# jwp3/async-multigrid

Measured on AMD Instinct MI355X. Metric: V-cycle iters/sec + fine-grid SpMV HBM GB/s, 512³ 7-pt Laplacian, 1/2/4/8 GPU, higher is better.
Workload: dtype f64

## Files before the change

### async-multigrid_amd/csrc/amg_api.cpp

```cpp
#include <algorithm>
#include <cmath>
#include <cstdlib>
#include <cstdint>
#include <cstring>
#include <mutex>
#include <vector>

#include "amg_async.h"

#include <csignal>
#include <execinfo.h>
#include <unistd.h>

namespace {
struct sigaction g_prev_segv, g_prev_bus, g_prev_abrt;
void amg_fault_trace(int sig, siginfo_t *si, void *uc)
{
   char msg[96];
   const int m = snprintf(msg, sizeof(msg), "[amg] signal %d at address %p, native backtrace:\n", sig, si->si_addr);
   if (m > 0) (void)!write(2, msg, (size_t)m);
   void *buf[64];
   const int n = backtrace(buf, 64);
   backtrace_symbols_fd(buf, n, 2);
   const struct sigaction &prev = sig == SIGSEGV ? g_prev_segv : sig == SIGBUS ? g_prev_bus : g_prev_abrt;
   if ((prev.sa_flags & SA_SIGINFO) && prev.sa_sigaction) {
      prev.sa_sigaction(sig, si, uc);
   } else if (prev.sa_handler != SIG_DFL && prev.sa_handler != SIG_IGN && prev.sa_handler) {
      prev.sa_handler(sig);
   }
   signal(sig, SIG_DFL);
   raise(sig);
}
__attribute__((constructor)) void amg_fault_trace_init()
{
   const char *e = std::getenv("AMG_SEGV_TRACE");
   if (!e || std::atoi(e) == 0) return;
   void *warm[4];
   (void)backtrace(warm, 4);
   struct sigaction sa;
   std::memset(&sa, 0, sizeof(sa));
   sa.sa_sigaction = amg_fault_trace;
   sa.sa_flags = SA_SIGINFO | SA_ONSTACK;
   sigaction(SIGSEGV, &sa, &g_prev_segv);
   sigaction(SIGBUS, &sa, &g_prev_bus);
   sigaction(SIGABRT, &sa, &g_prev_abrt);
}
}

static thread_local std::string g_last_error;

int amg_set_error(int code, const char *fmt, ...)
{
   char buf[1024];
   va_list ap;
   va_start(ap, fmt);
   vsnprintf(buf, sizeof(buf), fmt, ap);
   va_end(ap);
   g_last_error = buf;
   return code;
}

extern "C" const char *amg_last_error(void) { return g_last_error.c_str(); }
extern "C" int amg_version(void) { return 1; }

extern "C" void amg_opts_default(amg_opts *o)
{
   std::memset(o, 0, sizeof(*o));
   o->solver = AMG_MULT;
   o->smoother = AMG_JACOBI;
   o->num_pre_smooth_sweeps = 1;
   o->num_post_smooth_sweeps = 1;
   o->num_fine_smooth_sweeps = 1;
   o->num_coarse_smooth_sweeps = 1;
   o->smooth_weight = 1.0;
   o->num_cycles = 20;
   o->tol = 1e-9;
   o->check_resnorm = 1;
   o->cheby_flag = 0;
   o->num_threads = 1;
   o->jgs_block_rows = 64;
   o->reuse_outer_residual = 0;
   o->async_type = AMG_FULL_ASYNC;
   o->profile = 0;
   o->accel_type = AMG_NO_ACCEL;
   o->cheby_grid = 0;
   o->delay_type = AMG_DELAY_NONE;
   o->delay_usec = 0;
   o->delay_frac = 0.0;
   o->fail_iter = 0;
   o->delay_rank = -1;
   o->max_inflight = 1;
   o->async_comm_save_divisor = 1;
   o->sps_probability_type = AMG_SPS_EXPONENTIAL;
   o->sps_alpha = 1.0;
   o->sps_min_prob = 0.0;
   o->delay_level = -1;
}

extern "C" int amg_init(amg_ctx **out, int device, int nstreams)
{
   AMG_ARG(out, "amg_init: null out");
   int ndev = 0;
   AMG_HIP(hipGetDeviceCount(&ndev));
   AMG_ARG(device >= 0 && device < ndev, "amg_init: device %d of %d", device, ndev);
   AMG_HIP(hipSetDevice(device));
   amg_ctx *c = new amg_ctx();
   c->device = device;
   AMG_HIP(hipStreamCreateWithFlags(&c->stream, hipStreamNonBlocking));
   {
      int least = 0, greatest = 0;
      const char *v = std::getenv("AMG_COMM_PRIORITY");
      const bool hi = v && std::atoi(v) != 0;
      if (hi && hipDeviceGetStreamPriorityRange(&least, &greatest) == hipSuccess && greatest != least) {
         AMG_HIP(hipStreamCreateWithPriority(&c->comm_stream, hipStreamNonBlocking, greatest));
      } else {
         (void)hipGetLastError();
         AMG_HIP(hipStreamCreateWithFlags(&c->comm_stream, hipStreamNonBlocking));
      }
   }
   for (int i = 0; i < std::max(0, nstreams); i++) {
      hipStream_t s;
      AMG_HIP(hipStreamCreateWithFlags(&s, hipStreamNonBlocking));
      c->level_streams.push_back(s);
   }
   AMG_HIP(hipMalloc(&c->d_scalars, 8192 * sizeof(double)));
   AMG_HIP(hipMemset(c->d_scalars, 0, 8192 * sizeof(double)));
   AMG_HIP(hipMalloc(&c->d_err, 64));
   AMG_HIP(hipMemset(c->d_err, 0, 64));
   AMG_HIP(hipHostMalloc(&c->h_pinned, 1024 * sizeof(double)));
   hipDeviceProp_t prop;
   if (hipGetDeviceProperties(&prop, device) == hipSuccess) c->num_cus = prop.multiProcessorCount;
   if (hipDeviceGetAttribute(&c->wall_khz, hipDeviceAttributeWallClockRate, device) != hipSuccess || c->wall_khz <= 0)
      c->wall_khz = 100000;
   if (const char *v = std::getenv("AMG_VALUE_INDEX")) c->value_index = std::atoi(v) != 0;
   if (const char *v = std::getenv("AMG_DICT_INDEX")) c->dict_index = std::atoi(v) != 0;
   if (const char *v = std::getenv("AMG_ROW_PATTERN")) c->row_pattern = std::atoi(v) != 0;
   if (const char *v = std::getenv("AMG_PAIR_PATTERN")) c->pair_pattern = std::min(2, std::max(0, std::atoi(v)));
   if (const char *v = std::getenv("AMG_MASTER_PATTERN")) c->master_pattern = std::atoi(v) != 0;
   if (const char *v = std::getenv("AMG_PAIR_ANCHOR16")) c->pair_anchor16 = std::atoi(v) != 0;
   if (const char *v = std::getenv("AMG_PLANE_MARCH")) {
      c->plane_march = std::atoi(v) > 0;
      if (std::atoi(v) > 1) c->mz_zc = std::min(std::atoi(v), 64), c->mz_zc_auto = 0;
   }
   if (const char *v = std::getenv("AMG_PLANE_MARCH_XCD")) c->mz_xcd = std::atoi(v) != 0;
   if (const char *v = std::getenv("AMG_FUSE_TRANSFER")) c->fuse_transfer = std::atoi(v) != 0;
   if (const char *v = std::getenv("AMG_FUSE_XFER")) c->fuse_xfer = std::atoi(v) != 0;
   if (const char *v = std::getenv("AMG_GRAPHS")) c->graphs = std::atoi(v) != 0;
   if (const char *v = std::getenv("AMG_LONG_FORM")) c->long_form = std::max(0, std::min(2, std::atoi(v)));
   if (const char *v = std::getenv("AMG_LONG_XCD")) c->long_xcd = std::atoi(v) != 0;
   if (const char *v = std::getenv("AMG_OUTER_SLAB")) c->outer_slab = std::max(1, std::atoi(v));
   if (const char *v = std::getenv("AMG_FUSE_OUTER")) c->fuse_outer = std::max(0, std::min(3, std::atoi(v)));
   if (const char *v = std::getenv("AMG_FUSE_XFP_SLAB")) c->fuse_xfp_slab = std::atoi(v) != 0;
   if (const char *v = std::getenv("AMG_FUSE_PROLONG")) c->fuse_prolong = std::max(0, std::min(7, std::atoi(v)));
   if (const char *v = std::getenv("AMG_JGS_SMALL")) c->jgs_small = std::max(0, std::min(2, std::atoi(v)));
   if (const char *v = std::getenv("AMG_JGS_WAVE")) c->jgs_wave = std::max(0, std::min(3, std::atoi(v)));
   if (const char *v = std::getenv("AMG_JGS_FOLD")) c->jgs_fold = std::atoi(v) != 0;
   if (const char *v = std::getenv("AMG_BSR3")) c->bsr3 = std::max(0, std::min(std::atoi(v), 2));
   if (const char *v = std::getenv("AMG_BSR3_XS")) c->bsr3_xs = std::atoi(v) != 0;
   if (const char *v = std::getenv("AMG_MZ_EDGE")) c->mz_edge = std::atoi(v) != 0;
   if (const char *v = std::getenv("AMG_MZ27_OCC")) c->mz27_occ = std::max(-1, std::min(8, std::atoi(v)));
   if (const char *v = std::getenv("AMG_MZ_OCC")) c->mz_occ = std::max(-1, std::min(8, std::atoi(v)));
   if (const char *v = std::getenv("AMG_MZ_PF")) c->mz_pf = std::atoi(v) == 2 ? 2 : (std::atoi(v) == 1 ? 1 : 3);
   if (const char *v = std::getenv("AMG_MZ27_PF")) c->mz27_pf = std::atoi(v) == 1 ? 1 : (std::atoi(v) == 3 ? 3 : 2);
   if (const char *v = std::getenv("AMG_RR_LINES")) c->rr_lines = std::atoi(v) == 2 ? 2 : 1;
   if (const char *v = std::getenv("AMG_RR_OCC")) c->rr_occ = std::atoi(v);
   if (const char *v = std::getenv("AMG_RR_FPF")) c->rr_fpf = std::atoi(v);
   if (const char *v = std::getenv("AMG_RR_ZC")) c->rr_zc = std::max(0, std::min(std::atoi(v), 32));
   if (const char *v = std::getenv("AMG_RR_RING")) c->rr_ring = std::atoi(v) != 0;
   if (const char *v = std::getenv("AMG_MZ_NT")) c->mz_nt = std::atoi(v) & 3;
   if (const char *v = std::getenv("AMG_MZ_LINES")) c->mz_lines = std::atoi(v) == 4 ? 4 : std::atoi(v) == 2 ? 2 : 1;
   if (const char *v = std::getenv("AMG_MZ_LINES_GEMV"))
      c->mz_lines_gemv = std::atoi(v) == 4 ? 4 : std::atoi(v) == 2 ? 2 : 1;
   *out = c;
   return AMG_OK;
}

std::recursive_mutex &amg_teardown_mutex()
{
   static std::recursive_mutex m;
   return m;
}

extern "C" int amg_finalize(amg_ctx *c)
{
   if (!c) return AMG_OK;
   std::lock_guard<std::recursive_mutex> td(amg_teardown_mutex());
   hipSetDevice(c->device);
   hipStreamSynchronize(c->stream);
   if (c->comm_stream) hipStreamSynchronize(c->comm_stream);
   for (auto s : c->level_streams) {
      hipStreamSynchronize(s);
      hipStreamDestroy(s);
   }
   if (c->comm_stream) hipStreamDestroy(c->comm_stream);
   hipStreamDestroy(c->stream);
   hipFree(c->d_partials);
   hipFree(c->d_scalars);
   hipFree(c->d_err);
   hipHostFree(c->h_pinned);
   delete c;
   return AMG_OK;
}

extern "C" int amg_device_errors(amg_ctx *c, int *flags)
{
   AMG_ARG(c && flags, "amg_device_errors: null argument");
   int h[16];
   AMG_HIP(hipStreamSynchronize(c->stream));
   AMG_HIP(hipMemcpy(h, c->d_err, sizeof(h), hipMemcpyDeviceToHost));
   AMG_HIP(hipMemset(c->d_err, 0, sizeof(h)));
   *flags = h[0];
   return AMG_OK;
}

extern "C" int amg_sync(amg_ctx *c)
{
   AMG_ARG(c, "amg_sync: null ctx");
   AMG_HIP(hipStreamSynchronize(c->stream));
   return AMG_OK;
}

int amg_ctx_partials(amg_ctx *c, size_t n, double **out)
{
   if (n > c->partials_cap) {
      AMG_HIP(hipStreamSynchronize(c->stream));
      hipFree(c->d_partials);
      c->d_partials = nullptr;
      size_t cap = std::max<size_t>(n, 1 << 16);
      AMG_HIP(hipMalloc(&c->d_partials, cap * sizeof(double)));
      c->partials_cap = cap;
   }
   *out = c->d_partials;
   return AMG_OK;
}

static int mat_alloc(amg_ctx *c, int nrows, int ncols, long long nnz, amg_mat **out)
{
   amg_mat *A = new amg_mat();
   A->ctx = c;
   A->nrows = nrows;
   A->ncols = ncols;
   A->nnz = nnz;
   size_t np = (size_t)nnz + AMG_NNZ_PAD;
   hipError_t e = hipMalloc(&A->rowptr, ((size_t)nrows + 1) * sizeof(int));
   if (e == hipSuccess) e = hipMalloc(&A->col, np * sizeof(int));
   if (e == hipSuccess) e = hipMalloc(&A->val, np * sizeof(double));
   if (e == hipSuccess) e = hipMalloc(&A->diag, std::max(1, nrows) * sizeof(double));
   if (e != hipSuccess) {
      hipFree(A->rowptr); hipFree(A->col); hipFree(A->val); hipFree(A->diag);
      delete A;
      return amg_set_error(AMG_ERR_OOM, "amg_csr_register: device allocation of %lld nnz failed: %s",
                           nnz, hipGetErrorString(e));
   }
   AMG_HIP(hipMemsetAsync(A->col + nnz, 0, AMG_NNZ_PAD * sizeof(int), c->stream));
   AMG_HIP(hipMemsetAsync(A->val + nnz, 0, AMG_NNZ_PAD * sizeof(double), c->stream));
   *out = A;
   return AMG_OK;
}

static int build_value_index(amg_mat *A)
{
   amg_ctx *c = A->ctx;
   hipStream_t s = c->stream;
   constexpr int NS = 4096;
   unsigned long long *slots = nullptr;
   AMG_HIP(hipMalloc(&slots, NS * sizeof(unsigned long long) + 64));
   int *count = reinterpret_cast<int *>(slots + NS);
   AMG_HIP(hipMemsetAsync(slots, 0xff, NS * sizeof(unsigned long long), s));
   AMG_HIP(hipMemsetAsync(count, 0, sizeof(int), s));
   amgk::vi_collect(s, A->val, A->nnz, slots, NS, count);
   std::vector<unsigned long long> h(NS);
   int cnt = 0;
   AMG_HIP(hipMemcpyAsync(h.data(), slots, NS * sizeof(unsigned long long), hipMemcpyDeviceToHost, s));
   AMG_HIP(hipMemcpyAsync(&cnt, count, sizeof(int), hipMemcpyDeviceToHost, s));
   AMG_HIP(hipStreamSynchronize(s));
   if (cnt < 1 || cnt > 256) {
      hipFree(slots);
      return AMG_OK;
   }
   std::vector<unsigned long long> keys;
   for (auto k : h)
      if (k != ~0ULL) keys.push_back(k);
   std::sort(keys.begin(), keys.end());
   const int T = (int)keys.size();
   std::vector<double> tab(256, 0.0);
   std::memcpy(tab.data(), keys.data(), T * sizeof(double));
   hipError_t e = hipMalloc(&A->vidx, (size_t)A->nnz + 64);
   if (e == hipSuccess) e = hipMalloc(&A->vtab, 256 * sizeof(double));
   if (e != hipSuccess) {
      hipFree(A->vidx);
      hipFree(A->vtab);
      A->vidx = nullptr;
      A->vtab = nullptr;
      hipFree(slots);
      (void)hipGetLastError();
      return AMG_OK;
   }
   AMG_HIP(hipMemcpyAsync(slots, keys.data(), T * sizeof(unsigned long long), hipMemcpyHostToDevice, s));
   AMG_HIP(hipMemcpyAsync(A->vtab, tab.data(), 256 * sizeof(double), hipMemcpyHostToDevice, s));
   AMG_HIP(hipMemsetAsync(A->vidx + A->nnz, 0, 64, s));
   amgk::vi_encode(s, A->val, A->nnz, slots, T, A->vidx);
   AMG_HIP(hipStreamSynchronize(s));
   hipFree(slots);
   A->vi_n = T;
// ... 433 lines not shown
   A->mz_xlo = A->mz_xhi = -1;
}

int amg_mat_finish(amg_mat *A)
{
   amgk::extract_diag(A->ctx->stream, A);
   AMG_HIP(hipGetLastError());
   {
      int *d = nullptr;
      AMG_HIP(hipMalloc(&d, 2 * sizeof(int)));
      AMG_HIP(hipMemsetAsync(d, 0, 2 * sizeof(int), A->ctx->stream));
      amgk::row_max(A->ctx->stream, A, d);
      amgk::diag_uniform(A->ctx->stream, A, d + 1);
      int h[2] = {0, 0};
      double d0 = 0.0;
      hipError_t e = hipMemcpyAsync(h, d, 2 * sizeof(int), hipMemcpyDeviceToHost, A->ctx->stream);
      if (e == hipSuccess && A->nrows > 0)
         e = hipMemcpyAsync(&d0, A->diag, sizeof(double), hipMemcpyDeviceToHost, A->ctx->stream);
      if (e == hipSuccess) e = hipStreamSynchronize(A->ctx->stream);
      hipFree(d);
      if (e != hipSuccess) return amg_set_error(AMG_ERR_HIP, "amg_mat_finish: %s", hipGetErrorString(e));
      A->maxrow = h[0];
      A->diag_uni = A->nrows > 0 && h[1] == 0;
      A->diag_u = d0;
   }
   if (A->ctx->value_index && A->nnz > 0) AMG_TRY(build_value_index(A));
   if (A->ctx->dict_index && A->vidx) AMG_TRY(build_dict_index(A));
   if (A->ctx->row_pattern && A->didx) AMG_TRY(build_row_pattern(A));
   const bool pp = A->dc_maxrow <= 8 || A->nrows >= AMG_PP_LONG_MIN_ROWS || A->ctx->pair_pattern == 2;
   const bool try27 = !pp && A->ctx->plane_march && A->ctx->master_pattern;
   if (A->ctx->pair_pattern && A->rpat && A->dc_maxrow <= AMG_PP_MAXROW && (pp || try27))
      AMG_TRY(build_pair_pattern(A));
   if (A->ctx->master_pattern && A->ppat) AMG_TRY(build_master_pattern(A));
   if (try27 && A->ppat && !A->mz27 && !A->pbase) drop_pair_forms(A);
   return AMG_OK;
}

extern "C" int amg_set_row_pattern(amg_ctx *c, int enable)
{
   AMG_ARG(c, "amg_set_row_pattern: null context");
   c->knob_gen++;
   c->row_pattern = enable ? 1 : 0;
   return AMG_OK;
}

extern "C" int amg_mat_row_pattern(const amg_mat *A)
{
   return A ? A->rp_n : 0;
}

extern "C" int amg_set_pair_pattern(amg_ctx *c, int enable)
{
   AMG_ARG(c, "amg_set_pair_pattern: null context");
   c->knob_gen++;
   c->pair_pattern = enable < 0 ? 0 : enable > 2 ? 2 : enable;
   return AMG_OK;
}

extern "C" int amg_mat_pair_pattern(const amg_mat *A)
{
   return A ? A->pp_n : 0;
}

extern "C" int amg_set_pair_anchor16(amg_ctx *c, int enable)
{
   AMG_ARG(c, "amg_set_pair_anchor16: null context");
   c->knob_gen++;
   c->pair_anchor16 = enable ? 1 : 0;
   return AMG_OK;
}

extern "C" int amg_mat_pair_anchor16(const amg_mat *A)
{
   return (A && A->pdelta) ? 1 : 0;
}

extern "C" int amg_set_master_pattern(amg_ctx *c, int enable)
{
   AMG_ARG(c, "amg_set_master_pattern: null context");
   c->knob_gen++;
   c->master_pattern = enable ? 1 : 0;
   return AMG_OK;
}

extern "C" int amg_mat_master_pattern(const amg_mat *A)
{
   return A ? A->mp_J * (A->mp_uni ? -1 : 1) : 0;
}

extern "C" int amg_set_plane_march(amg_ctx *c, int enable, int zc, int xcd)
{
   AMG_ARG(c, "amg_set_plane_march: null context");
   AMG_ARG(zc >= -1 && zc <= 64, "amg_set_plane_march: planes per chunk %d outside [1, 64] (0: keep, -1: auto)",
           zc);
   c->knob_gen++;
   c->plane_march = enable ? 1 : 0;
   if (zc > 0) c->mz_zc = zc, c->mz_zc_auto = 0;
   if (zc == -1) c->mz_zc = 16, c->mz_zc_auto = 1;
   if (xcd >= 0) c->mz_xcd = xcd ? 1 : 0;
   return AMG_OK;
}

extern "C" int amg_set_jgs_wave(amg_ctx *c, int enable)
{
   AMG_ARG(c, "amg_set_jgs_wave: null context");
   c->knob_gen++;
   c->jgs_wave = std::max(0, std::min(3, enable));
   return AMG_OK;
}

extern "C" int amg_set_jgs_small(amg_ctx *c, int form)
{
   AMG_ARG(c, "amg_set_jgs_small: null context");
   c->knob_gen++;
   c->jgs_small = std::max(0, std::min(2, form));
   return AMG_OK;
}

extern "C" int amg_set_jgs_fold(amg_ctx *c, int enable)
{
   AMG_ARG(c, "amg_set_jgs_fold: null context");
   c->knob_gen++;
   c->jgs_fold = enable != 0;
   return AMG_OK;
}

extern "C" int amg_set_fuse_prolong(amg_ctx *c, int enable)
{
   AMG_ARG(c, "amg_set_fuse_prolong: null context");
   c->knob_gen++;
   c->fuse_prolong = std::max(0, std::min(7, enable));
   return AMG_OK;
}

extern "C" int amg_set_march_lines(amg_ctx *c, int lines)
{
   AMG_ARG(c && (lines == 1 || lines == 2 || lines == 4), "amg_set_march_lines: lines must be 1, 2 or 4");
   c->knob_gen++;
   c->mz_lines = lines;
   c->mz_lines_gemv = lines;
   return AMG_OK;
}

extern "C" int amg_set_march_lines_gemv(amg_ctx *c, int lines)
{
   AMG_ARG(c && (lines == 1 || lines == 2 || lines == 4), "amg_set_march_lines_gemv: lines must be 1, 2 or 4");
   c->knob_gen++;
   c->mz_lines_gemv = lines;
   return AMG_OK;
}

extern "C" int amg_set_fuse_outer(amg_ctx *c, int mode)
{
   AMG_ARG(c && mode >= 0 && mode <= 3, "amg_set_fuse_outer: mode 0, 1, 2 or 3");
   c->knob_gen++;
   c->fuse_outer = mode;
   return AMG_OK;
}

extern "C" int amg_set_outer_slab(amg_ctx *c, int planes)
{
   AMG_ARG(c && planes >= 1, "amg_set_outer_slab: planes must be >= 1");
   c->knob_gen++;
   c->outer_slab = planes;
   return AMG_OK;
}

extern "C" int amg_set_long_form(amg_ctx *c, int form, int xcd)
{
   AMG_ARG(c && form >= 0 && form <= 2, "amg_set_long_form: form 0, 1 or 2");
   c->knob_gen++;
   c->long_form = form;
   c->long_xcd = xcd != 0;
   return AMG_OK;
}

extern "C" int amg_set_graphs(amg_ctx *c, int enable)
{
   AMG_ARG(c, "amg_set_graphs: null context");
   c->knob_gen++;
   c->graphs = enable != 0;
   return AMG_OK;
}

extern "C" int amg_set_march_tuning(amg_ctx *c, int mz_pf, int mz27_pf, int mz_occ, int mz27_occ)
{
   AMG_ARG(c, "amg_set_march_tuning: null context");
   AMG_ARG(mz_pf == -2 || (mz_pf >= 1 && mz_pf <= 3), "amg_set_march_tuning: 7-pt prefetch distance %d", mz_pf);
   AMG_ARG(mz27_pf == -2 || mz27_pf == 1 || mz27_pf == 2 || mz27_pf == 3,
           "amg_set_march_tuning: 27-pt prefetch distance %d (3: the LDS plane ring)",
           mz27_pf);
   AMG_ARG(mz_occ >= -2 && mz_occ <= 8 && mz27_occ >= -2 && mz27_occ <= 8,
           "amg_set_march_tuning: occupancy %d / %d outside [-1, 8]", mz_occ, mz27_occ);
   c->knob_gen++;
   if (mz_pf != -2) c->mz_pf = mz_pf;
   if (mz27_pf != -2) c->mz27_pf = mz27_pf;
   if (mz_occ != -2) c->mz_occ = mz_occ;
   if (mz27_occ != -2) c->mz27_occ = mz27_occ;
   return AMG_OK;
}

extern "C" int amg_set_fuse_transfer(amg_ctx *c, int enable)
{
   AMG_ARG(c, "amg_set_fuse_transfer: null context");
   c->knob_gen++;
   c->fuse_transfer = enable ? 1 : 0;
   return AMG_OK;
}

extern "C" int amg_mat_plane_march(const amg_mat *A)
{
   return A ? A->mz_P : 0;
}

extern "C" int amg_mat_march_points(const amg_mat *A)
{
   return (A && A->mz_P) ? (A->mz27 ? 27 : 7) : 0;
}

extern "C" int amg_set_dict_index(amg_ctx *c, int enable)
{
   AMG_ARG(c, "amg_set_dict_index: null context");
   c->knob_gen++;
   c->dict_index = enable ? 1 : 0;
   return AMG_OK;
}

extern "C" int amg_mat_dict_index(const amg_mat *A)
{
   return A ? A->dc_n : 0;
}

extern "C" int amg_set_value_index(amg_ctx *c, int enable)
{
   AMG_ARG(c, "amg_set_value_index: null context");
   c->knob_gen++;
   c->value_index = enable ? 1 : 0;
   return AMG_OK;
}

extern "C" int amg_mat_value_index(const amg_mat *A)
{
   return A ? A->vi_n : 0;
}

int amg_mat_create_device(amg_ctx *c, int nrows, int ncols, long long nnz, amg_mat **out)
{
   return mat_alloc(c, nrows, ncols, nnz, out);
}

static int build_bsr3(amg_mat *A, const int *rowptr, const int *col, const double *val)
{
   const int n = A->nrows, nb = n / 3;
   if (!A->ctx->bsr3 || n % 3 || n != A->ncols || !A->diag_first || n < 3 || A->nnz < 24LL * n) return AMG_OK;
   std::vector<int> bptr(nb + 1, 0), bdiag(nb, -1), bcol;
   std::vector<unsigned char> mode(nb, 1);
   std::vector<long long> src;
   std::vector<int> js;
   long long blocked = 0;
   for (int t = 0; t < nb; t++) {
      bptr[t + 1] = bptr[t];
      const int r0 = 3 * t;
      const int len = rowptr[r0 + 1] - rowptr[r0];
      if (len < 3 || len % 3) continue;
      bool ok = true;
      js.clear();
      for (int c = 0; c < 3 && ok; c++) {
         const int r = r0 + c, b = rowptr[r], e = rowptr[r + 1];
         ok = e - b == len && col[b] == r;
         int prev = -1, k = b + 1;
         std::vector<int> cols;
         cols.reserve(len);
         bool ins = false;
         for (int q = 0; q < len - 1 && ok; q++, k++) {
            const int cc = col[k];
            if (!ins && r < cc) cols.push_back(r), ins = true;
            ok = cc > prev && cc != r;
            prev = cc;
            cols.push_back(cc);
         }
         if (!ins) cols.push_back(r);
         for (int q = 0; q < len && ok; q += 3) {
            ok = cols[q] % 3 == 0 && cols[q + 1] == cols[q] + 1 && cols[q + 2] == cols[q] + 2;
            if (ok && c == 0) js.push_back(cols[q] / 3);
            if (ok && c > 0) ok = js[q / 3] == cols[q] / 3;
         }
      }
      if (!ok) continue;
      mode[t] = 0;
      blocked++;
      for (size_t q = 0; q < js.size(); q++) {
         if (js[q] == t) bdiag[t] = bptr[t + 1];
         bcol.push_back(js[q]);
         bptr[t + 1]++;
      }
      if (bdiag[t] < 0) return AMG_OK;
      const size_t base = src.size();
      src.resize(base + js.size() * 9, -1);
      for (int c = 0; c < 3; c++) {
         const int r = r0 + c, b = rowptr[r], e = rowptr[r + 1];
         for (int k = b; k < e; k++) {
            const int j = col[k] / 3, cc = col[k] % 3;
            const size_t q = std::lower_bound(js.begin(), js.end(), j) - js.begin();
            src[base + q * 9 + 3 * c + cc] = k;
         }
      }
   }
// ... 619 lines not shown
```

### async-multigrid_amd/csrc/amg_internal.h

```cpp
#pragma once

#include <hip/hip_runtime.h>

#include <cstdarg>
#include <cstdint>
#include <cstdio>
#include <functional>
#include <string>
#include <limits>
#include <vector>

#include "amg_mi355x.h"

int amg_set_error(int code, const char *fmt, ...);

#define AMG_HIP(call)                                                                      \
   do {                                                                                    \
      hipError_t _e = (call);                                                              \
      if (_e != hipSuccess)                                                                \
         return amg_set_error(AMG_ERR_HIP, "%s:%d %s -> %s", __FILE__, __LINE__, #call,   \
                              hipGetErrorString(_e));                                      \
   } while (0)

#define AMG_TRY(call)                                                                      \
   do {                                                                                    \
      int _s = (call);                                                                     \
      if (_s != AMG_OK) return _s;                                                         \
   } while (0)

#define AMG_ARG(cond, ...)                                                                 \
   do {                                                                                    \
      if (!(cond)) return amg_set_error(AMG_ERR_ARG, __VA_ARGS__);                         \
   } while (0)

constexpr int AMG_TILE_ROWS = 256;
constexpr int AMG_CHUNK = 2048;
constexpr int AMG_NNZ_PAD = 8;
constexpr int AMG_DC_MAXROW = 32;
constexpr int AMG_RP_STRIDE = 36;
constexpr int AMG_PP_MAXROW = 32;
constexpr int AMG_PP_LDS = 32 * 1024;
constexpr int AMG_PP_LONG_MIN_ROWS = 1 << 22;
inline int amg_pp_stride(int maxrow) { return 1 + 2 * (maxrow <= 8 ? 8 : AMG_PP_MAXROW); }

constexpr int AMG_PP_NDA = 16;
constexpr int AMG_PP_DA0 = 8;
constexpr int AMG_PP_NK = 256 * 257 * AMG_PP_NDA;
constexpr double AMG_PP_MAXFILL = 1.15;
constexpr int AMG_RPP_OPT = 2;
constexpr int AMG_MP_MAXJ = 32;
constexpr int AMG_MP_LDS = 48 * 1024;

struct amg_transport;

struct amg_ctx {
   amg_transport *xport = nullptr;
   long long replicate_rows = 1LL << 18;
   int device = 0;
   hipStream_t stream = nullptr;
   std::vector<hipStream_t> level_streams;
   hipStream_t comm_stream = nullptr;
   double *d_partials = nullptr;
   size_t partials_cap = 0;
   double *d_scalars = nullptr;
   int *d_err = nullptr;
   double *h_pinned = nullptr;
   int num_cus = 256;
   int wall_khz = 100000;
   int value_index = 1;
   int dict_index = 1;
   int row_pattern = 1;
   int pair_pattern = 1;
   int master_pattern = 1;
   int pair_anchor16 = 0;
   int plane_march = 1;
   int mz_zc = 16;
   int mz_edge = 1;
   int mz_zc_auto = 1;
   int mz27_occ = -1;
   int mz_occ = 0;
   int mz_pf = 3;
   int mz27_pf = 2;
   int mz_xcd = 1;
   int fuse_transfer = 1;
   int bsr3 = 2;
   unsigned knob_gen = 0;
   int graphs = 0;
   int fuse_xfer = 1;
   int fuse_xfp_slab = 0;
   int fuse_prolong = 0;
   int bsr3_xs = 1;
   int fuse_outer = 0;
   int outer_slab = 32;
   int rr_lines = 1;
   int mz_lines = 1;
   int mz_lines_gemv = 2;
   int mz_nt = 0;
   int rr_ring = 0;
   int rr_occ = 0;
   int rr_fpf = 0;
   int long_form = 0;
   int long_xcd = 1;
   int rr_zc = 0;
   int jgs_wave = 1;
   int jgs_small = 2;
   int jgs_fold = 0;
};

struct amg_mat {
   amg_ctx *ctx = nullptr;
   int nrows = 0, ncols = 0;
   long long nnz = 0;
   int *rowptr = nullptr;
   int *col = nullptr;
   double *val = nullptr;
   double *diag = nullptr;
   int diag_first = 1;
   int maxrow = -1;
   amg_mat *trans = nullptr;
   unsigned char *vidx = nullptr;
   double *vtab = nullptr;
   int vi_n = 0;
   unsigned char *didx = nullptr;
   int *doff = nullptr;
   double *dval = nullptr;
   int *danch = nullptr;
   int dc_n = 0;
   int dc_maxrow = 0;
   unsigned char *rpat = nullptr;
   unsigned char *ptab = nullptr;
   int rp_n = 0;
   unsigned char *ppat = nullptr;
   unsigned int *pptab = nullptr;
   int pp_n = 0;
   int pp_stride = 0;
   int pp_centre0 = 0;
   int *pbase = nullptr;
   unsigned short *pdelta = nullptr;
   int mp_J = 0;
   int mp_uni = 0;
   int diag_uni = 0;
   double diag_u = 0.0;
   int mp_off[AMG_MP_MAXJ] = {};
   double mp_val[AMG_MP_MAXJ] = {};
   unsigned long long *mpmask = nullptr;
   double *mpval = nullptr;
   int mz_P = 0, mz_S = 0;
   int mz27 = 0;
   int mz_dom = -1;
   double mz_domval[27] = {};
   int mz_xlo = -1, mz_xhi = -1;
   double mz_hival[27] = {};
   int bsr3 = 0;
   int bsl = 21;
   long long *soff = nullptr;
   int *bcol = nullptr, *bdiag = nullptr;
   unsigned char *bmode = nullptr;
   unsigned int *bvi = nullptr;
   double *bval = nullptr;
};

struct amg_vec {
   amg_ctx *ctx = nullptr;
   int n = 0;
   double *d = nullptr;
   bool owns = true;
};

int amg_ctx_partials(amg_ctx *ctx, size_t n, double **out);
int amg_mat_create_device(amg_ctx *c, int nrows, int ncols, long long nnz, amg_mat **out);
int amg_mat_finish(amg_mat *A);
int amg_hier_subcycle(amg_hier *H, hipStream_t s, const double *f_dev, const double **u_dev);
int amg_hier_reset(amg_hier *H);

namespace amgk {

struct Gemv {
   int init;
   int negacc;
   int scale;
   double alpha, temp;
};
Gemv gemv_mode(double alpha, double beta);

void spgemv(hipStream_t s, const amg_mat *A, const double *x, const double *b, const Gemv &g,
            double *y, int rb, int re, double *partials);
void residual_fsub(hipStream_t s, const amg_mat *A, const double *x, const double *b, double *y, double *r, int n);
int tile_blocks(int rb, int re);

void jacobi_sweep(hipStream_t s, const amg_mat *A, const double *f, const double *x,
                  const double *l1, double omega, double *out, int rb, int re);
void residual_jacobi(hipStream_t s, const amg_mat *A, const double *f, const double *x,
                     const double *l1, double omega, double *r, double *unext, int rb, int re,
                     double *partials);
bool mz_sweep_outer_ok(const amg_mat *A);
void mz_sweep_outer(hipStream_t s, const amg_mat *A, const double *f, const double *u, double *u1out,
                    double *rout, double *unext, double omega, double *partials);
void jacobi_zero(hipStream_t s, const double *diag, const double *f, const double *l1,
                 double omega, double *u, int rb, int re, int variant);
void jacobi_from_residual(hipStream_t s, const double *diag, const double *r, const double *l1,
                          double omega, double *u, int rb, int re);
bool hybrid_jgs(hipStream_t s, const amg_mat *A, const double *f, double *u, const double *u_prev,
                const int *d_blk, int nblk, const double *diag_scale, double weight, int zero,
                int reverse, double *apply_u = nullptr, double *apply_priv = nullptr,
                unsigned long long *stamp = nullptr);
void row_max(hipStream_t s, const amg_mat *A, int *d_out);
void async_gs(hipStream_t s, const amg_mat *A, const double *f, double *u, const int *d_blk, int nblk,
              int sweeps, int semi, int reverse);
struct GeoT {
   double w[27];
   int nx, ny, nz;
};
void geo_check(hipStream_t s, const amg_mat *M, int mode, const GeoT &g, int *bad, int rb = 0, int re = -1,
               long long row_g0 = 0, long long col_g0 = 0);
struct ZeroGuess {
   const double *d = nullptr;
   double w = 0.0;
   double *u = nullptr;
   long long lo = 0, hi = -1;
   int *err = nullptr;
};
void mz_residual_restrict(hipStream_t s, const amg_mat *A, const double *f, const double *u, const GeoT &g,
                          const double *wdev, double *fc, int Kb = 0, int Ke = -1, int fz0 = 0, int cz0 = 0,
                          ZeroGuess zg = ZeroGuess());
void geo_restrict(hipStream_t s, const GeoT &g, const double *wdev, const double *r, double *fc, int Kb = 0,
                  int Ke = -1, int fz0 = 0, int cz0 = 0, ZeroGuess zg = ZeroGuess());
void geo_prolong(hipStream_t s, const GeoT &g, const double *wdev, const double *e, double *u, int zb = 0,
                 int ze = -1, int fz0 = 0, int cz0 = 0, int assign = 0);
void dmem_scale(hipStream_t s, const double *diag, const double *l1, double omega, double *sc, double *nsc, int n);
void delay(hipStream_t s, double usec, int wall_khz);
void mz_prolong_sweep(hipStream_t s, const amg_mat *A, const double *f, const double *u, const double *ec,
                      const GeoT &g, const double *wdev, const double *l1, double omega, double *uout);
void mz_xfer_restrict(hipStream_t s, const amg_mat *A, const double *r, const GeoT &g, const double *wdev,
                      double omega, double *rc, int Kb = 0, int Ke = -1, int fz0 = 0, int cz0 = 0);
void mz_xfer_prolong(hipStream_t s, const amg_mat *A, const double *ec, const GeoT &g, const double *wdev,
                     double omega, int mode, double *out, double *u_priv, int zlo = 0, int zhi = -1, int fz0 = 0,
                     int cz0 = 0, unsigned long long *stamp = nullptr);
void matvec_t_chunked(hipStream_t s, const amg_mat *AT, const double *x, double *y, int n_src,
                      int T);

void vcopy(hipStream_t s, const double *x, double *y, int rb, int re);
void vset(hipStream_t s, double *y, double a, int rb, int re);
void vaxpy(hipStream_t s, double a, const double *x, double *y, int rb, int re);
void vivaxpy(hipStream_t s, const double *x, const double *sc, double *y, int rb, int re);
void vscale(hipStream_t s, double a, double *y, int rb, int re);
// ... 70 lines not shown
```

### async-multigrid_amd/csrc/amg_kernels.hip

```cpp
#include "amg_internal.h"

#include <mutex>
#include <unordered_map>

#include <algorithm>
#include <type_traits>

namespace amgk {

template <int V>
using int_c = std::integral_constant<int, V>;
template <int V>
constexpr int_c<V> otherwise{};

template <class F>
static inline void pick_bool(bool b, F &&f)
{
   if (b) f(std::true_type{});
   else f(std::false_type{});
}

template <int... Vs, int D, class F>
static inline void pick_int(int v, int_c<D>, F &&f)
{
// ... 3209 lines not shown
      } else {
         const v2d q = jac_div2(v2d{omega * res.x, omega * res.y}, a, dq, rq);
         v = v2d{(a.x != 0.0) ? xi.x + q.x : xi.x, (a.y != 0.0) ? xi.y + q.y : xi.y};
      }
      st2(unext + i, v, nt);
      return res;
   }
};

constexpr int AMG_MZF_NL = 2;
constexpr int AMG_MZF_NT = AMG_MZF_NL + 2;

template <bool STORE_U, int MINB, int PD = 1>
__global__ __launch_bounds__(256 * AMG_MZF_NT) __attribute__((amdgpu_waves_per_eu(MINB * 4))) void
mz_sweep_outer_kernel(
   const unsigned char *__restrict__ ppat, const unsigned long long *__restrict__ mmask_g, int np, MpSten Sv,
   const double *__restrict__ f, const double *__restrict__ u, double *__restrict__ u1out,
   double *__restrict__ rout, double *__restrict__ unext, double omega, int P, int nz, int zc, int npb, int xcd,
   double *__restrict__ partials, double dq, double rq)
{
   constexpr int NL = AMG_MZF_NL, NT = AMG_MZF_NT, S = 512;
   __shared__ unsigned long long mtab[256];
   __shared__ v2d ring[2][NT][256];
   __shared__ double red[AMG_MZ_MAXZC * NL * 8];
   const int tid = (int)threadIdx.x, team = tid >> 8, lt = tid & 255, lane = tid & 63;
   if (tid < np) mtab[tid] = mmask_g[tid];
   const int G = (int)gridDim.x;
   int lg = (int)blockIdx.x;
   if (xcd && (G & 7) == 0) lg = (lg & 7) * (G >> 3) + (lg >> 3);
   const int pblk = lg % npb, chunk = lg / npb;
   const int k0 = chunk * zc, k1 = min(k0 + zc, nz);
   const int ny = P / S;
   const int y = pblk * NL - 1 + team;
   const bool inner = team >= 1 && team <= NL;
   const int ly = y < 0 ? 0 : (y >= ny ? ny - 1 : y);
   const unsigned pos = (unsigned)(ly * S + 2 * lt);
   const unsigned Nu = (unsigned)((long long)nz * P);
   const double a0 = Sv.val[0];
   const v2d a2{a0, a0};
   auto ldp = [&](int k) { return (k >= 0 && k < nz) ? ld2u(u, (unsigned)k * P + pos) : v2d{0.0, 0.0}; };
   v2d xm = ldp(k0 - 2), xc = ldp(k0 - 1), xq = ldp(k0), xn = PD == 2 ? ldp(k0 + 1) : v2d{0.0, 0.0};
   struct PlaneIn {
      v2d ym, yp, fv;
      double e;
      int pid;
   };
   auto fetch = [&](int k, PlaneIn &in) {
      const int kk = k < 0 ? 0 : (k >= nz ? nz - 1 : k);
      const unsigned row = (unsigned)kk * P + pos;
      in.ym = ld2u(u, row >= (unsigned)S ? row - S : 0u);
      const unsigned rp = row + (unsigned)S;
      in.yp = ld2u(u, rp + 2 <= Nu ? rp : Nu - 2);
      in.fv = ld2u(f, row);
      in.pid = ppat[row >> 1];
      in.e = 0.0;
      if (lane == 0 && row > 0) in.e = ld1u(u, row - 1);
      if (lane == 63 && row + 2 < Nu) in.e = ld1u(u, row + 2);
   };
   PlaneIn cur, nx1{};
   fetch(k0 - 1, cur);
   if (PD == 2 && k0 <= k1) fetch(k0, nx1);
   v2d wm{0.0, 0.0}, wc{0.0, 0.0}, fm{0.0, 0.0};
   int pidm = 0;
   __syncthreads();
   for (int k = k0 - 1; k <= k1; k++) {
      const bool s1 = k >= 0 && k < nz;
      const v2d xnn = ldp(k + 1 + PD);
      v2d w1{0.0, 0.0};
      if (s1) {
         double lft = __shfl_up(xc.y, 1, 64);
         double rgt = __shfl_down(xc.x, 1, 64);
         if (lane == 0) lft = cur.e;
         if (lane == 63) rgt = cur.e;
         const unsigned long long mk = mtab[cur.pid];
         v2d xv[7];
         xv[0] = xc;
         xv[1] = xm;
         xv[2] = cur.ym;
         xv[3] = v2d{lft, xc.x};
         xv[4] = v2d{xc.y, rgt};
         xv[5] = cur.yp;
         xv[6] = xq;
         const v2d acc = mz_acc7<1, true>(cur.fv, xv, mk, Sv, nullptr);
         const v2d q = jac_div2(v2d{omega * acc.x, omega * acc.y}, a2, dq, rq);
         w1 = v2d{(a0 != 0.0) ? xc.x + q.x : xc.x, (a0 != 0.0) ? xc.y + q.y : xc.y};
         if (STORE_U && inner && y < ny && k >= k0 && k < k1)
            *reinterpret_cast<v2du *>(u1out + (size_t)((unsigned)k * P + pos)) = w1;
      }
      ring[k & 1][team][lt] = w1;
      const v2d fk = cur.fv;
      const int pidk = cur.pid;
      PlaneIn nxt{};
      if (k + PD <= k1) fetch(k + PD, nxt);
      const int km = k - 1;
      if (km >= k0 && km < k1) {
         if (inner && y < ny) {
            const v2d *rg = ring[km & 1][0];
            const double *rl = reinterpret_cast<const double *>(ring[km & 1][team]);
            const double lft = rl[lt > 0 ? 2 * lt - 1 : 0];
            const double rgt = rl[lt < 255 ? 2 * lt + 2 : 511];
            const unsigned long long mk = mtab[pidm];
            v2d xv[7];
            xv[0] = wc;
            xv[1] = wm;
            xv[2] = rg[(team - 1) * 256 + lt];
            xv[3] = v2d{lft, wc.x};
            xv[4] = v2d{wc.y, rgt};
            xv[5] = rg[(team + 1) * 256 + lt];
            xv[6] = s1 ? w1 : v2d{0.0, 0.0};
            const v2d res = mz_acc7<1, true>(fm, xv, mk, Sv, nullptr);
            const unsigned row = (unsigned)km * P + pos;
            if (rout) *reinterpret_cast<v2du *>(rout + (size_t)row) = res;
            const v2d q = jac_div2(v2d{omega * res.x, omega * res.y}, a2, dq, rq);
            const v2d v{(a0 != 0.0) ? wc.x + q.x : wc.x, (a0 != 0.0) ? wc.y + q.y : wc.y};
            *reinterpret_cast<v2du *>(unext + (size_t)row) = v;
            if (partials) {
               double a = res.x * res.x, b = res.y * res.y;
#pragma unroll
               for (int off = 16; off > 0; off >>= 1) {
                  a += __shfl_down(a, off, 32);
                  b += __shfl_down(b, off, 32);
               }
               if ((lt & 31) == 0) red[((km - k0) * NL + (team - 1)) * 8 + (lt >> 5)] = a + b;
            }
         }
      }
      __syncthreads();
      wm = wc;
      wc = w1;
      fm = fk;
      pidm = pidk;
      xm = xc;
      xc = xq;
      if (PD == 2) {
         xq = xn;
         xn = xnn;
         cur = nx1;
         nx1 = nxt;
      } else {
         xq = xnn;
         cur = nxt;
      }
   }
   if (partials) {
      for (int w = tid; w < 2 * NL * (k1 - k0); w += 256 * NT) {
         const int it = w / (2 * NL), i = (w >> 1) % NL, h = w & 1;
         const int yl = pblk * NL + i;
         const double *g = red + (it * NL + i) * 8 + 4 * h;
         partials[((long long)(k0 + it) * P + (long long)yl * S) / 256 + h] = ((g[0] + g[1]) + g[2]) + g[3];
      }
   }
}

bool mz_sweep_outer_ok(const amg_mat *A)
{
   return A->mz_P && !A->mz27 && A->mp_uni && A->mz_S == 512 && A->mz_P % 512 == 0 &&
          (A->mz_P / 512) % AMG_MZF_NL == 0 && A->ppat && A->mpmask;
}

static bool fast_div_of(const amg_mat *A, double *d, double *y);

void mz_sweep_outer(hipStream_t s, const amg_mat *A, const double *f, const double *u, double *u1out,
                    double *rout, double *unext, double omega, double *partials)
{
   const MpSten Sv = mp_sten(A);
   const int P = A->mz_P, nz = A->nrows / P;
   const int npb = P / (512 * AMG_MZF_NL);
   int zc = std::max(1, std::min(A->ctx->mz_zc, AMG_MZ_MAXZC));
   if (A->ctx->mz_zc_auto) zc = (int)std::max(1LL, std::min((long long)zc, (long long)nz * npb / 1024));
   const int nch = (nz + zc - 1) / zc;
   static const int occ2 = [] {
      const char *e = std::getenv("AMG_FUSE_OUTER_OCC");
      return e && std::atoi(e) == 2;
   }();
   static const int pd = [] {
      const char *e = std::getenv("AMG_FUSE_OUTER_PD");
      return e && std::atoi(e) == 2 ? 2 : 1;
   }();
   double dq = 0.0, rq = 0.0;
   if (!fast_div_of(A, &dq, &rq)) dq = rq = 0.0;
   pick_bool(u1out != nullptr, [&](auto store) {
      pick_int<2>(occ2 ? 2 : 1, otherwise<1>, [&](auto minb) {
         pick_int<2>(pd, otherwise<1>, [&](auto pdc) {
            mz_sweep_outer_kernel<decltype(store)::value, decltype(minb)::value, decltype(pdc)::value>
               <<<npb * nch, 256 * AMG_MZF_NT, 0, s>>>(A->ppat, A->mpmask, A->pp_n, Sv, f, u, u1out, rout, unext, omega,
                                                       P, nz, zc, npb, A->ctx->mz_xcd, partials, dq, rq);
         });
      });
   });
}

__device__ __forceinline__ const double *epi_pf_vec(const EpiJacobi &e) { return e.x; }
__device__ __forceinline__ const double *epi_pf_vec(const EpiL1Jacobi &e) { return e.x; }
__device__ __forceinline__ const double *epi_pf_vec(const EpiResJacobi &e) { return e.x; }

template <class Cfg>
static inline int cfg_blocks(int rb, int re)
{
   constexpr int T = 256 * Cfg::rpt;
   return (re - rb + T - 1) / T;
}

int tile_blocks(int rb, int re) { return cfg_blocks<ProdCfg>(rb, re); }

Gemv gemv_mode(double alpha, double beta)
{
   Gemv g;
   const double temp = beta / alpha;
   const int acase = (alpha == 1) ? 0 : (alpha == -1) ? 1 : 2;
   if (temp == 0)
      g.init = 0;
   else if (temp == -1)
      g.init = (acase == 1) ? 1 : 2;
   else if (temp == 1)
      g.init = (acase == 1) ? 2 : 1;
   else
      g.init = (acase == 1) ? 4 : 3;
   g.negacc = (acase == 1);
   g.scale = (acase == 2);
   g.alpha = alpha;
   g.temp = temp;
   return g;
}

template <int NEG, bool NEED_DIAG, class Epi, int U = 4>
__global__ __launch_bounds__(256) void bsr3_row_kernel(const long long *__restrict__ soff,
                                                       const int *__restrict__ bcol, const int *__restrict__ bdiag,
                                                       const unsigned char *__restrict__ bcnt,
                                                       const unsigned int *__restrict__ bvi,
                                                       const double *__restrict__ vtab_g,
                                                       const int *__restrict__ rowptr, const int *__restrict__ col,
                                                       const double *__restrict__ val, const double *__restrict__ x,
                                                       int t0, int t1, Epi epi)
{
   __shared__ double vtab[256];
   vtab[threadIdx.x] = vtab_g[threadIdx.x];
   __syncthreads();
   const int lane = threadIdx.x & 63, wave = threadIdx.x >> 6;
   const int sl = t0 / 64 + (int)blockIdx.x * 4 + wave;
   const int t = sl * 64 + lane;
   if (t < t0 || t >= t1) return;
   double acc[3], xi[3], a[3];
   auto madd = [&](double &ac, double v, double xv) { ac = NEG ? ac - v * xv : ac + v * xv; };
#pragma unroll
   for (int c = 0; c < 3; c++) {
      acc[c] = epi.init(3 * t + c);
      xi[c] = x[3 * t + c];
      a[c] = 0.0;
   }
   const int cnt = bcnt[t];
   if (cnt == 0) {
#pragma unroll
      for (int c = 0; c < 3; c++) {
         const int i = 3 * t + c, b = rowptr[i], e = rowptr[i + 1];
         if (NEED_DIAG) a[c] = b < e ? val[b] : 0.0;
         for (int k = b; k < e; k++) madd(acc[c], val[k], x[col[k]]);
      }
   } else {
      const long long base = soff[sl] + lane;
      const int kd = bdiag[t];
      {
         const unsigned int *w = bvi + (base + 64LL * kd) * 3;
#pragma unroll
         for (int c = 0; c < 3; c++) {
            a[c] = vtab[(w[c] >> (8 * c)) & 0xff];
            madd(acc[c], a[c], xi[c]);
         }
      }
      for (int kc = 0; kc < cnt; kc += U) {
         int jj[U];
         unsigned int wv[U][3];
#pragma unroll
         for (int u = 0; u < U; u++) {
            const long long sp = base + 64LL * min(kc + u, cnt - 1);
            jj[u] = bcol[sp];
#pragma unroll
            for (int c = 0; c < 3; c++) wv[u][c] = bvi[sp * 3 + c];
         }
         double xv[U][3];
#pragma unroll
         for (int u = 0; u < U; u++)
#pragma unroll
            for (int cc = 0; cc < 3; cc++) xv[u][cc] = x[3 * (size_t)jj[u] + cc];
#pragma unroll
         for (int u = 0; u < U; u++) {
            const int k = kc + u;
            if (k >= cnt) break;
#pragma unroll
            for (int c = 0; c < 3; c++)
#pragma unroll
               for (int cc = 0; cc < 3; cc++)
                  if (k != kd || c != cc) madd(acc[c], vtab[(wv[u][c] >> (8 * cc)) & 0xff], xv[u][cc]);
         }
      }
   }
#pragma unroll
   for (int c = 0; c < 3; c++)
      epi.finish(3 * t + c, acc[c], a[c], (pf_is_x<Epi>::value && epi_pf_vec(epi) == x) ? xi[c] : epi.pf(3 * t + c));
}

template <int NEG, bool NEED_DIAG, class Epi, bool VI, bool XS = false, int U = 9>
__global__ __launch_bounds__(256) void bsr3_kernel(const long long *__restrict__ soff, const int *__restrict__ bcol,
                                                   const int *__restrict__ bdiag,
                                                   const unsigned char *__restrict__ bcnt,
                                                   const unsigned int *__restrict__ bvi,
                                                   const double *__restrict__ bval, const double *__restrict__ vtab_g,
                                                   const int *__restrict__ rowptr, const int *__restrict__ col,
                                                   const double *__restrict__ val, const double *__restrict__ x,
                                                   int t0, int t1, Epi epi)
{
   __shared__ double vtab[VI ? 256 : 1];
   if (VI) vtab[threadIdx.x] = vtab_g[threadIdx.x];
   if (VI) __syncthreads();
   const int lane = threadIdx.x & 63, wave = threadIdx.x >> 6;
   if (lane >= 63) return;
   const int sl = t0 / 21 + (int)blockIdx.x * 4 + wave, q = lane / 3, c = lane % 3;
   const int t = sl * 21 + q;
   if (t < t0 || t >= t1) return;
   const int i = 3 * t + c;
// ... 2333 lines not shown
```

Before: 335.2.

## Add register-resident two-sweep Jacobi+residual plane-march kernel and enable by default

Adds a new fuse_outer mode 4 and makes it the default. It marches z-planes of two y-lines per block with a one-line halo kept in registers and LDS. Each plane gets a first Jacobi sweep, then the residual and a second Jacobi update of the previous plane are computed from the fresh values, so the intermediate iterate never round-trips through HBM. The trade-off is redundant halo-line computation and higher register pressure (waves_per_eu 3), and the new kernel replaces the existing outer-sweep path for all matrices that qualify.

```diff
diff --git a/async-multigrid_amd/csrc/amg_api.cpp b/async-multigrid_amd/csrc/amg_api.cpp
--- a/async-multigrid_amd/csrc/amg_api.cpp
+++ b/async-multigrid_amd/csrc/amg_api.cpp
@@ -149,7 +149,7 @@
    if (const char *v = std::getenv("AMG_LONG_FORM")) c->long_form = std::max(0, std::min(2, std::atoi(v)));
    if (const char *v = std::getenv("AMG_LONG_XCD")) c->long_xcd = std::atoi(v) != 0;
    if (const char *v = std::getenv("AMG_OUTER_SLAB")) c->outer_slab = std::max(1, std::atoi(v));
-   if (const char *v = std::getenv("AMG_FUSE_OUTER")) c->fuse_outer = std::max(0, std::min(3, std::atoi(v)));
+   if (const char *v = std::getenv("AMG_FUSE_OUTER")) c->fuse_outer = std::max(0, std::min(4, std::atoi(v)));
    if (const char *v = std::getenv("AMG_FUSE_XFP_SLAB")) c->fuse_xfp_slab = std::atoi(v) != 0;
    if (const char *v = std::getenv("AMG_FUSE_PROLONG")) c->fuse_prolong = std::max(0, std::min(7, std::atoi(v)));
    if (const char *v = std::getenv("AMG_JGS_SMALL")) c->jgs_small = std::max(0, std::min(2, std::atoi(v)));
@@ -889,7 +889,7 @@
 
 extern "C" int amg_set_fuse_outer(amg_ctx *c, int mode)
 {
-   AMG_ARG(c && mode >= 0 && mode <= 3, "amg_set_fuse_outer: mode 0, 1, 2 or 3");
+   AMG_ARG(c && mode >= 0 && mode <= 4, "amg_set_fuse_outer: mode 0, 1, 2, 3 or 4");
    c->knob_gen++;
    c->fuse_outer = mode;
    return AMG_OK;
diff --git a/async-multigrid_amd/csrc/amg_internal.h b/async-multigrid_amd/csrc/amg_internal.h
--- a/async-multigrid_amd/csrc/amg_internal.h
+++ b/async-multigrid_amd/csrc/amg_internal.h
@@ -90,7 +90,7 @@
    int fuse_xfp_slab = 0;
    int fuse_prolong = 0;
    int bsr3_xs = 1;
-   int fuse_outer = 0;
+   int fuse_outer = 4;
    int outer_slab = 32;
    int rr_lines = 1;
    int mz_lines = 1;
diff --git a/async-multigrid_amd/csrc/amg_kernels.hip b/async-multigrid_amd/csrc/amg_kernels.hip
--- a/async-multigrid_amd/csrc/amg_kernels.hip
+++ b/async-multigrid_amd/csrc/amg_kernels.hip
@@ -3385,6 +3385,172 @@
    }
 }
 
+constexpr int AMG_MZR_NL = 2;
+
+template <int NL, bool STORE_U, bool STORE_R>
+__global__ __launch_bounds__(256) __attribute__((amdgpu_waves_per_eu(3))) void mz_two_sweep_kernel(
+   const unsigned char *__restrict__ ppat, const unsigned long long *__restrict__ mmask_g, int np, MpSten Sv,
+   const double *__restrict__ f, const double *__restrict__ u, double *__restrict__ u1out,
+   double *__restrict__ rout, double *__restrict__ unext, double omega, int P, int nz, int zc, int npb, int xcd,
+   double *__restrict__ partials, double dq, double rq)
+{
+   constexpr int NS = NL + 2, S = 512;
+   __shared__ unsigned long long mtab[256];
+   __shared__ double ue[2][NS][4][2];
+   __shared__ double we[2][NL][4][2];
+   __shared__ double red[AMG_MZ_MAXZC * NL * 8];
+   const int tid = (int)threadIdx.x, lane = tid & 63, wv = tid >> 6;
+   if (tid < np) mtab[tid] = mmask_g[tid];
+   const int G = (int)gridDim.x;
+   int lg = (int)blockIdx.x;
+   if (xcd && (G & 7) == 0) lg = (lg & 7) * (G >> 3) + (lg >> 3);
+   const int pblk = lg % npb, chunk = lg / npb;
+   const int k0 = chunk * zc, k1 = min(k0 + zc, nz);
+   const int ny = P / S, y0 = pblk * NL;
+   auto lofs = [&](int y) { return (unsigned)((y < 0 ? 0 : (y >= ny ? ny - 1 : y)) * S); };
+   unsigned lof[NS];
+#pragma unroll
+   for (int j = 0; j < NS; j++) lof[j] = lofs(y0 - 1 + j);
+   const unsigned lofm = lofs(y0 - 2), lofp = lofs(y0 + NL + 1);
+   const unsigned lo = 2u * (unsigned)tid;
+   const double a0 = Sv.val[0];
+   const v2d a2{a0, a0};
+   auto ldp = [&](int k, int j) {
+      return (k >= 0 && k < nz) ? ld2u(u + ((size_t)k * P + lof[j]), lo) : v2d{0.0, 0.0};
+   };
+   auto edge = [&](const double (&e)[4][2]) {
+      double v = 0.0;
+      if (lane == 0 && wv > 0) v = e[wv - 1][1];
+      if (lane == 63 && wv < 3) v = e[wv + 1][0];
+      return v;
+   };
+   v2d um[NS], uc[NS], uq[NS];
+#pragma unroll
+   for (int j = 0; j < NS; j++) {
+      um[j] = ldp(k0 - 2, j);
+      uc[j] = ldp(k0 - 1, j);
+      uq[j] = ldp(k0, j);
+      if (lane == 0) ue[(k0 - 1) & 1][j][wv][0] = uc[j].x;
+      if (lane == 63) ue[(k0 - 1) & 1][j][wv][1] = uc[j].y;
+   }
+   v2d wm[NL], wc[NS], fm[NL];
+   int pidm[NL];
+#pragma unroll
+   for (int j = 0; j < NS; j++) wc[j] = v2d{0.0, 0.0};
+#pragma unroll
+   for (int i = 0; i < NL; i++) {
+      wm[i] = fm[i] = v2d{0.0, 0.0};
+      pidm[i] = 0;
+   }
+   __syncthreads();
+   for (int k = k0 - 1; k <= k1; k++) {
+      const bool s1 = k >= 0 && k < nz;
+      const size_t base = (size_t)(k < 0 ? 0 : (k >= nz ? nz - 1 : k)) * P;
+      const v2d ym = ld2u(u + (base + lofm), lo), yp = ld2u(u + (base + lofp), lo);
+      v2d fv[NS], un[NS];
+      int pid[NS];
+#pragma unroll
+      for (int j = 0; j < NS; j++) {
+         fv[j] = ld2u(f + (base + lof[j]), lo);
+         pid[j] = (ppat + ((base + lof[j]) >> 1))[tid];
+      }
+#pragma unroll
+      for (int j = 0; j < NS; j++) {
+         if (lane == 0) ue[(k + 1) & 1][j][wv][0] = uq[j].x;
+         if (lane == 63) ue[(k + 1) & 1][j][wv][1] = uq[j].y;
+      }
+      v2d w1[NS];
+#pragma unroll
+      for (int j = 0; j < NS; j++) {
+         w1[j] = v2d{0.0, 0.0};
+         if (s1) {
+            const double e = edge(ue[k & 1][j]);
+            double lft = __shfl_up(uc[j].y, 1, 64);
+            double rgt = __shfl_down(uc[j].x, 1, 64);
+            if (lane == 0) lft = e;
+            if (lane == 63) rgt = e;
+            const unsigned long long mk = mtab[pid[j]];
+            v2d xv[7];
+            xv[0] = uc[j];
+            xv[1] = um[j];
+            xv[2] = j == 0 ? ym : uc[j == 0 ? 0 : j - 1];
+            xv[3] = v2d{lft, uc[j].x};
+            xv[4] = v2d{uc[j].y, rgt};
+            xv[5] = j == NS - 1 ? yp : uc[j == NS - 1 ? 0 : j + 1];
+            xv[6] = uq[j];
+            const v2d acc = mz_acc7<1, true>(fv[j], xv, mk, Sv, nullptr);
+            const v2d q = jac_div2(v2d{omega * acc.x, omega * acc.y}, a2, dq, rq);
+            w1[j] = v2d{(a0 != 0.0) ? uc[j].x + q.x : uc[j].x, (a0 != 0.0) ? uc[j].y + q.y : uc[j].y};
+            if (j >= 1 && j <= NL) {
+               if (STORE_U && k >= k0 && k < k1)
+                  *reinterpret_cast<v2du *>(u1out + ((size_t)k * P + lof[j]) + lo) = w1[j];
+               if (lane == 0) we[k & 1][j - 1][wv][0] = w1[j].x;
+               if (lane == 63) we[k & 1][j - 1][wv][1] = w1[j].y;
+            }
+         }
+      }
+#pragma unroll
+      for (int j = 0; j < NS; j++) un[j] = k < k1 ? ldp(k + 2, j) : v2d{0.0, 0.0};
+      const int km = k - 1;
+      if (km >= k0) {
+#pragma unroll
+         for (int i = 0; i < NL; i++) {
+            const int j = i + 1;
+            const double e = edge(we[km & 1][i]);
+            double lft = __shfl_up(wc[j].y, 1, 64);
+            double rgt = __shfl_down(wc[j].x, 1, 64);
+            if (lane == 0) lft = e;
+            if (lane == 63) rgt = e;
+            const unsigned long long mk = mtab[pidm[i]];
+            v2d xv[7];
+            xv[0] = wc[j];
+            xv[1] = wm[i];
+            xv[2] = wc[j - 1];
+            xv[3] = v2d{lft, wc[j].x};
+            xv[4] = v2d{wc[j].y, rgt};
+            xv[5] = wc[j + 1];
+            xv[6] = w1[j];
+            const v2d res = mz_acc7<1, true>(fm[i], xv, mk, Sv, nullptr);
+            const size_t row = (size_t)km * P + lof[j];
+            if (STORE_R) *reinterpret_cast<v2du *>(rout + row + lo) = res;
+            const v2d q = jac_div2(v2d{omega * res.x, omega * res.y}, a2, dq, rq);
+            const v2d v{(a0 != 0.0) ? wc[j].x + q.x : wc[j].x, (a0 != 0.0) ? wc[j].y + q.y : wc[j].y};
+            *reinterpret_cast<v2du *>(unext + row + lo) = v;
+            if (partials) {
+               double a = res.x * res.x, b = res.y * res.y;
+#pragma unroll
+               for (int off = 16; off > 0; off >>= 1) {
+                  a += __shfl_down(a, off, 32);
+                  b += __shfl_down(b, off, 32);
+               }
+               if ((tid & 31) == 0) red[((km - k0) * NL + i) * 8 + (tid >> 5)] = a + b;
+            }
+         }
+      }
+      __syncthreads();
+#pragma unroll
+      for (int i = 0; i < NL; i++) {
+         wm[i] = wc[i + 1];
+         fm[i] = fv[i + 1];
+         pidm[i] = pid[i + 1];
+      }
+#pragma unroll
+      for (int j = 0; j < NS; j++) {
+         wc[j] = w1[j];
+         um[j] = uc[j];
+         uc[j] = uq[j];
+         uq[j] = un[j];
+      }
+   }
+   if (partials) {
+      for (int w = tid; w < 2 * NL * (k1 - k0); w += 256) {
+         const int it = w / (2 * NL), i = (w >> 1) % NL, h = w & 1;
+         const double *g = red + (it * NL + i) * 8 + 4 * h;
+         partials[((long long)(k0 + it) * P + (long long)(y0 + i) * S) / 256 + h] = ((g[0] + g[1]) + g[2]) + g[3];
+      }
+   }
+}
+
 bool mz_sweep_outer_ok(const amg_mat *A)
 {
    return A->mz_P && !A->mz27 && A->mp_uni && A->mz_S == 512 && A->mz_P % 512 == 0 &&
@@ -3398,6 +3564,20 @@
 {
    const MpSten Sv = mp_sten(A);
    const int P = A->mz_P, nz = A->nrows / P;
+   if (A->ctx->fuse_outer == 4) {
+      double dq = 0.0, rq = 0.0;
+      if (!fast_div_of(A, &dq, &rq)) dq = rq = 0.0;
+      const int npb = P / (512 * AMG_MZR_NL);
+      pick_bool(u1out != nullptr, [&](auto store) {
+         pick_bool(rout != nullptr, [&](auto res) {
+            auto *fn = mz_two_sweep_kernel<AMG_MZR_NL, decltype(store)::value, decltype(res)::value>;
+            const int zc = occ_chunk(A, nz, npb, -1, (const void *)fn), nch = (nz + zc - 1) / zc;
+            fn<<<npb * nch, 256, 0, s>>>(A->ppat, A->mpmask, A->pp_n, Sv, f, u, u1out, rout, unext, omega, P, nz, zc,
+                                         npb, A->ctx->mz_xcd, partials, dq, rq);
+         });
+      });
+      return;
+   }
    const int npb = P / (512 * AMG_MZF_NL);
    int zc = std::max(1, std::min(A->ctx->mz_zc, AMG_MZ_MAXZC));
    if (A->ctx->mz_zc_auto) zc = (int)std::max(1LL, std::min((long long)zc, (long long)nz * npb / 1024));
```

Result: faster. 377.4 (median of 6 runs) (+12.6%).
